# KKKSQJ/DeepLearning

Measured on NVIDIA H100. Metric: images/sec (ResNet-50 training step), higher is better.
Workload: dtype bf16

## Files before the change

### deeplearning_b200/csrc/abi_conv.cu

```cuda
#include <string.h>
#include "../../include/b200cls.h"
#include "conv_gemm.cuh"
#include "conv1x1_stream.cuh"
#include "conv_tap64.cuh"
#include "host_utils.h"
#include "wgrad_gemm.cuh"

using namespace b200;

namespace {

constexpr uint32_t kFwdDescLbo = 16, kFwdDescSbo = 1024;
constexpr uint32_t kWgDescLbo = 8192, kWgDescSbo = 1024, kWgDescKstep = 2048;

struct Box3 {
  int b1, b2, b3;
};

Box3 choose_box(long long d1, long long d2, long long d3, int P) {
  Box3 best{P, 1, 1};
  double best_cost = -1;
  for (int b1 = 1; b1 <= P; b1 <<= 1) {
    for (int b2 = 1; b1 * b2 <= P; b2 <<= 1) {
      const int b3 = P / (b1 * b2);
// ... 127 lines not shown
    }
  } else {
    *qb = Box3{bx.b1 / 4, 1, 1};
    for (int q = 0; q < 4; ++q) o1[q] = q * (bx.b1 / 4);
  }
}

int setup_output(ConvGemmParams& p, const View& dv, int N, int out_f32, const View* auxv) {
  const long long d1 = dv.dims[1], d2 = dv.dims[2], d3 = dv.dims[3];
  const Box3 bx = choose_box(d1, d2, d3, 128);
  p.box1 = bx.b1, p.box2 = bx.b2, p.box3 = bx.b3;
  p.dim1 = static_cast<int>(d1), p.dim2 = static_cast<int>(d2), p.dim3 = static_cast<int>(d3);
  p.tiles1 = static_cast<int>((d1 + bx.b1 - 1) / bx.b1);
  p.tiles2 = static_cast<int>((d2 + bx.b2 - 1) / bx.b2);
  p.tiles3 = static_cast<int>((d3 + bx.b3 - 1) / bx.b3);
  p.N = N;
  const int BN = N <= 64 ? 64 : 128;
  p.n_tiles = (N + BN - 1) / BN;
  Box3 qb;
  quarter_box(bx, &qb, p.qoff1, p.qoff2, p.qoff3);
  p.out_f32 = out_f32;
  if (dv.base != nullptr) {
    uint32_t box[4] = {out_f32 ? 32u : 64u, (uint32_t)qb.b1, (uint32_t)qb.b2, (uint32_t)qb.b3};
    int rc = out_f32 ? encode_tmap_f32(&p.d_map, dv.base, 4, dv.dims, dv.strides, box)
                     : encode_tmap_bf16(&p.d_map, dv.base, 4, dv.dims, dv.strides, box);
    if (rc) return rc;
  }
  p.has_aux_out = 0;
  if (auxv != nullptr) {
    uint32_t box[4] = {64u, (uint32_t)qb.b1, (uint32_t)qb.b2, (uint32_t)qb.b3};
    int rc = encode_tmap_bf16(&p.aux_map, auxv->base, 4, auxv->dims, auxv->strides, box);
    if (rc) return rc;
    p.has_aux_out = 1;
  }
  return OK;
}
Box3 box_of(const ConvGemmParams& p) { return Box3{p.box1, p.box2, p.box3}; }

bool bn_mask_complete(const b200_bn_mask_t* m) { return m->x_raw && m->scale && m->shift && m->stats; }
void set_bn_mask(ConvGemmParams& p, const b200_bn_mask_t* m, const View& dv) {
  p.mask_in = static_cast<const __nv_bfloat16*>(m->x_raw);
  p.ms1 = static_cast<long long>(dv.strides[1]);
  p.ms2 = static_cast<long long>(dv.strides[2]);
  p.ms3 = static_cast<long long>(dv.strides[3]);
  p.bn_scale = m->scale, p.bn_shift = m->shift, p.stats = m->stats;
}

int conv_grid(int tiles, int n_tiles, bool stats) {
  int grid = tiles < device_sm_count() ? tiles : device_sm_count();
  if (stats) grid = grid / n_tiles * n_tiles;
  return grid;
}

template <int BLOCK_N, int EPI>
int launch_conv_gemm_epi(const ConvGemmParams& q, int grid, cudaStream_t st) {
  using Cfg = ConvGemmCfg<BLOCK_N>;
  static bool configured = false;
  if (!configured) {
    B200_CHECK_CUDA(cudaFuncSetAttribute(conv_gemm_kernel<BLOCK_N, EPI>, cudaFuncAttributeMaxDynamicSharedMemorySize,
                                         Cfg::SMEM_BYTES));
    configured = true;
  }
  B200_CHECK_CUDA(launch_pdl(conv_gemm_kernel<BLOCK_N, EPI>, dim3(grid), dim3(Cfg::THREADS), Cfg::SMEM_BYTES, st, q));
  B200_LAUNCHED();
  return OK;
}

int epilogue_flags(const ConvGemmParams& p) {
  int f = 0;
  if (p.bias) f |= kEpiBias;
  if (p.colscale) f |= kEpiColscale;
  f |= (p.act & 3) << kEpiActShift;
  if (p.residual) f |= p.res_f32 ? kEpiResF32 : kEpiResBf16;
  if (p.has_aux_out) f |= kEpiAux;
  if (p.out_f32) f |= kEpiOutF32;
  if (p.out_direct) f |= kEpiDirect;
  if (p.stats) f |= kEpiStats;
  if (p.rowscale) f |= kEpiRowscale;
  if (p.affine) f = (f & ~(kEpiBias | kEpiColscale)) | kEpiAffine;
  if (p.mask_in) f |= p.bn_scale ? kEpiBnMask : kEpiMask;
  if (p.bn_scale) f &= ~kEpiStats;
  return f;
}

#define B200_EPI_LIST(X)                                                                                  \
  X(kEpiStats)                                              \
  X(0)                                                      \
  X(kEpiResBf16)                                            \
  X(kEpiBias)                                               \
  X(kEpiBias | kEpiResF32 | kEpiOutF32)                     \
  X(kEpiBias | kEpiColscale | kEpiResF32 | kEpiOutF32)      \
  X(kEpiBias | (2 << kEpiActShift) | kEpiAux)               \
  X(3 << kEpiActShift)                                      \
  X((3 << kEpiActShift) | kEpiStats)                        \
  X(kEpiOutF32)                                             \
  X(kEpiBias | kEpiOutF32)                                  \
  X(kEpiAffine | kEpiResBf16 | (1 << kEpiActShift))        \
  X(kEpiAffine | (1 << kEpiActShift))                      \
  X(kEpiAffine)                                            \
  X(kEpiMask | kEpiResBf16 | kEpiStats)                    \
  X(kEpiBnMask)                                            \
  X(kEpiBnMask | kEpiBias)

bool tap64_ok(const ConvGemmParams& p) {
  const int f = epilogue_flags(p);
  return p.N == 64 && p.n_tiles == 1 && p.k_per_tap == 64 && p.k_blocks_per_tap == 1 && !p.var_taps && !p.chan_window &&
         p.num_taps >= 2 && p.num_taps <= 9 && (f == 0 || f == kEpiStats) && p.dim1 % p.box1 == 0 && p.dim2 % p.box2 == 0 &&
         p.dim3 % p.box3 == 0;
}
template <bool kStats>
int launch_tap64(const ConvGemmParams& q, int grid, cudaStream_t st) {
  static bool configured = false;
  if (!configured) {
    B200_CHECK_CUDA(cudaFuncSetAttribute(conv_tap64_kernel<kStats>, cudaFuncAttributeMaxDynamicSharedMemorySize, kTap64SmemBytes));
    configured = true;
  }
  B200_CHECK_CUDA(launch_pdl(conv_tap64_kernel<kStats>, dim3(grid), dim3(384), kTap64SmemBytes, st, q));
  B200_LAUNCHED();
  return OK;
}

template <int BLOCK_N>
int launch_conv_gemm(const ConvGemmParams& p, cudaStream_t st) {
  const int tiles = p.tiles1 * p.tiles2 * p.tiles3 * p.n_tiles;
  const int grid = conv_grid(tiles, p.n_tiles, p.stats != nullptr);
  B200_REQUIRE(grid > 0, "conv_gemm: %d channel blocks exceed the SM count (BN statistics need grid %% n_tiles == 0)", p.n_tiles);
  ConvGemmParams q = p;
  q.desc_lbo = kFwdDescLbo;
  q.desc_sbo = kFwdDescSbo;
  if constexpr (BLOCK_N == 64) {
    if (tap64_ok(p)) return p.stats != nullptr ? launch_tap64<true>(q, grid, st) : launch_tap64<false>(q, grid, st);
  }
  switch (epilogue_flags(p)) {
#define B200_EPI_CASE(F) \
  case (F):              \
    return launch_conv_gemm_epi<BLOCK_N, (F)>(q, grid, st);
    B200_EPI_LIST(B200_EPI_CASE)
#undef B200_EPI_CASE
    default:
      return launch_conv_gemm_epi<BLOCK_N, kEpiGeneric>(q, grid, st);
  }
}


bool stream_ok(long long pixels, int K, int N) {
  return (K == 64 || K == 128 || K == 256) && N % 256 == 0 && pixels % 128 == 0 && pixels / 128 < (1LL << 30);
}
int stream_grid(long long pixels, int N) {
  const int n_tiles = N / 256;
  const long long items = pixels / 128 * n_tiles;
  int grid = items < device_sm_count() ? static_cast<int>(items) : device_sm_count();
  return grid / n_tiles * n_tiles;
}

template <int KB, int MODE>
int launch_stream(const StreamParams& q, int grid, cudaStream_t st) {
  using Cfg = StreamCfg<KB, MODE>;
  static bool configured = false;
  if (!configured) {
    B200_CHECK_CUDA(cudaFuncSetAttribute(conv1x1_stream_kernel<KB, MODE>, cudaFuncAttributeMaxDynamicSharedMemorySize,
                                         Cfg::SMEM_BYTES));
    configured = true;
  }
  B200_CHECK_CUDA(launch_pdl(conv1x1_stream_kernel<KB, MODE>, dim3(grid), dim3(Cfg::THREADS), Cfg::SMEM_BYTES, st, q));
  B200_LAUNCHED();
  return OK;
}

int run_stream(int mode, const void* a, const void* w, void* out, const void* res, const void* mask, const float* scale,
               const float* shift, float* stats, long long pixels, int K, int N, cudaStream_t st) {
  StreamParams q;
  memset(&q, 0, sizeof(q));
  int rc;
  if ((rc = encode_matrix(&q.a_map, a, K, pixels, 128))) return rc;
  if ((rc = encode_matrix(&q.b_map, w, K, N, 256))) return rc;
  if ((rc = encode_matrix(&q.out_map, out, N, pixels, 16))) return rc;
  if (res != nullptr && (rc = encode_matrix(&q.res_map, res, N, pixels, 16))) return rc;
  if (mask != nullptr && (rc = encode_matrix(&q.mask_map, mask, N, pixels, 16))) return rc;
  q.m_tiles = static_cast<int>(pixels / 128);
  q.n_tiles = N / 256;
  q.N = N;
  q.scale = scale, q.shift = shift, q.stats = stats;
  const int grid = stream_grid(pixels, N);
// ... 172 lines not shown
  const int n_tiles = (Cout + BN - 1) / BN;
  const long long tiles = m_tiles * n_tiles;
  const int grid = conv_grid(tiles > (1 << 30) ? (1 << 30) : static_cast<int>(tiles), n_tiles, true);
  return grid / n_tiles * (BN == 64 ? 8 : 4);
}

int b200_conv2d_fwd_stats_rows(int B, int H, int W, int Cout, int ksize, int stride) {
  return fwd_stats_rows(B, H, W, Cout, ksize, stride, block_n_for(Cout));
}

static int conv_fwd(const void* x, const void* w, void* y, int B, int H, int W, int Cin, int Cout, int ksize, int stride,
                    float* stats, const float* bias, int act, const void* residual, float* out_f32, long long ld_out,
                    const float* bn_scale, const float* bn_shift, int y_f32, int Cg, void* stream) {
  B200_REQUIRE(ksize == 1 || ksize == 3 || (ksize == 2 && stride == 2), "conv2d_fwd: ksize %d / stride %d unsupported", ksize, stride);
  B200_REQUIRE(stride == 1 || stride == 2, "conv2d_fwd: stride %d unsupported (1 or 2)", stride);
  B200_REQUIRE(Cin % 8 == 0 && Cout % 8 == 0, "conv2d_fwd: Cin=%d / Cout=%d must be multiples of 8", Cin, Cout);
  B200_REQUIRE(B > 0 && H > 0 && W > 0, "conv2d_fwd: empty input");
  B200_REQUIRE(stride == 1 || (H >= 2 && W >= 2), "conv2d_fwd: stride-2 needs H,W >= 2");
  B200_REQUIRE(out_f32 == nullptr || (ksize == 1 && stride == 1), "conv2d_fwd: fp32 output only for 1x1/s1");
  B200_REQUIRE((bn_scale == nullptr) == (bn_shift == nullptr), "conv2d_fwd: bn_scale and bn_shift go together");
  B200_REQUIRE(bn_scale == nullptr || (Cout % 64 == 0 && bias == nullptr && stats == nullptr && out_f32 == nullptr && act <= 1 && !y_f32),
               "conv2d_fwd + folded BN: Cout=%d must be a multiple of 64, no bias / statistics / fp32 output", Cout);
  cudaStream_t st = static_cast<cudaStream_t>(stream);
  const int Ho = out_dim(H, ksize, stride), Wo = out_dim(W, ksize, stride);
  ConvGemmParams p;
  memset(&p, 0, sizeof(p));
  int rc;
  View dv = act_view(y, B, Ho, Wo, Cout, ksize == 1 && stride == 1);
  if (out_f32 != nullptr) dv.base = nullptr;
  if ((rc = setup_output(p, dv, Cout, y_f32, nullptr))) return rc;
  const int BN = Cg ? 64 : block_n_for(Cout);
  p.n_tiles = (Cout + BN - 1) / BN;
  p.chan_window = Cg ? 1 : 0;
  p.k_per_tap = Cg ? 64 : Cin;
  p.k_blocks_per_tap = Cg ? 1 : (Cin + 63) / 64;
  p.num_taps = ksize * ksize;
  if ((rc = encode_taps(p, p.a_maps, x, B, H, W, Cin, ksize, stride, box_of(p)))) return rc;
  for (int t = 0; t < p.num_taps; ++t) p.tap_w[t] = static_cast<int8_t>(t);
  if ((rc = encode_matrix(&p.b_map, w, static_cast<long long>(p.num_taps) * p.k_per_tap, Cout, BN))) return rc;
  p.stats = stats;
  p.bias = bias;
  p.act = act;
  p.residual = residual;
  p.rs1 = static_cast<long long>(dv.strides[1]);
  p.rs2 = static_cast<long long>(dv.strides[2]);
  p.rs3 = static_cast<long long>(dv.strides[3]);
  p.out_direct = out_f32;
  p.ld_out = ld_out;
  if (bn_scale != nullptr) {
    p.affine = 1;
    p.colscale = bn_scale;
    p.bias = bn_shift;
  }
  return Cg ? launch_conv_gemm<64>(p, st) : dispatch_conv_gemm(p, Cout, st);
}

int b200_conv2d_fwd(const void* x, const void* w, void* y, int B, int H, int W, int Cin, int Cout, int ksize, int stride,
                    float* stats, const float* bias, int act, const void* residual, float* out_f32, long long ld_out,
                    const float* bn_scale, const float* bn_shift, void* stream) {
  return conv_fwd(x, w, y, B, H, W, Cin, Cout, ksize, stride, stats, bias, act, residual, out_f32, ld_out, bn_scale, bn_shift,
                  0, 0, stream);
}

int b200_conv2d_fwd_f32(const void* x, const void* w, float* y, int B, int H, int W, int Cin, int Cout, int ksize,
                        int stride, const float* bias, void* stream) {
  return conv_fwd(x, w, y, B, H, W, Cin, Cout, ksize, stride, nullptr, bias, 0, nullptr, nullptr, 0, nullptr, nullptr, 1, 0,
                  stream);
}

static int conv_dgrad(const void* dy, const void* wd, void* dx, int B, int H, int W, int Cin, int Cout, int ksize,
                      int stride, const void* residual, const b200_bn_mask_t* bn_mask, int Cg, void* stream) {
  B200_REQUIRE(ksize == 1 || ksize == 3 || (ksize == 2 && stride == 2), "conv2d_dgrad: ksize %d / stride %d unsupported", ksize, stride);
  B200_REQUIRE(stride == 1 || stride == 2, "conv2d_dgrad: stride %d unsupported", stride);
  B200_REQUIRE(Cin % 8 == 0 && Cout % 8 == 0, "conv2d_dgrad: Cin=%d / Cout=%d must be multiples of 8", Cin, Cout);
  B200_REQUIRE(bn_mask == nullptr || (stride == 1 && Cin % 64 == 0 && bn_mask_complete(bn_mask)),
               "conv2d_dgrad: the fused BatchNorm-backward reduce needs stride 1, Cin %% 64 == 0 and every bn_mask field "
               "(Cin=%d, stride=%d)", Cin, stride);
  cudaStream_t st = static_cast<cudaStream_t>(stream);
  const int Ho = out_dim(H, ksize, stride), Wo = out_dim(W, ksize, stride);
  const bool flat = (ksize == 1 && stride == 1);
  const int BN = Cg ? 64 : block_n_for(Cin);
  const int k_per_tap = Cg ? 64 : Cout;
  int rc;
  CUtensorMap b_map;
  if ((rc = encode_matrix(&b_map, wd, static_cast<long long>(ksize * ksize) * k_per_tap, Cin, BN))) return rc;
  const int nphase = (stride == 2 && ksize >= 2) ? 2 : 1;
  for (int ph = 0; ph < nphase; ++ph) {
    for (int pw = 0; pw < nphase; ++pw) {
      ConvGemmParams p;
      memset(&p, 0, sizeof(p));
      p.b_map = b_map;
      View dv = flat ? make_flat_view(dx, static_cast<long long>(B) * H * W, Cin)
                     : make_view(dx, B, H, W, Cin, stride, ph, pw);
      if ((rc = setup_output(p, dv, Cin, 0, nullptr))) return rc;
      p.n_tiles = (Cin + BN - 1) / BN;
      p.chan_window = Cg ? 1 : 0;
      p.k_per_tap = k_per_tap;
      p.k_blocks_per_tap = Cg ? 1 : (Cout + 63) / 64;
      if ((rc = encode_view(&p.a_maps[0], act_view(dy, B, Ho, Wo, Cout, flat), box_of(p)))) return rc;
      for (int i = 1; i < 4; ++i) p.a_maps[i] = p.a_maps[0];
      int nt = 0;
      if (ksize == 1) {
        p.tap_map[0] = 0, p.tap_o1[0] = 0, p.tap_o2[0] = 0, p.tap_w[0] = 0;
        nt = 1;
      } else if (stride == 1) {
        for (int kh = 0; kh < 3; ++kh)
          for (int kw = 0; kw < 3; ++kw) {
            p.tap_map[nt] = 0;
            p.tap_o1[nt] = static_cast<int8_t>(1 - kw);
            p.tap_o2[nt] = static_cast<int8_t>(1 - kh);
            p.tap_w[nt] = static_cast<int8_t>(kh * 3 + kw);
            ++nt;
          }
      } else if (ksize == 2) {
        p.tap_map[0] = 0, p.tap_o1[0] = 0, p.tap_o2[0] = 0;
        p.tap_w[0] = static_cast<int8_t>(ph * 2 + pw);
        nt = 1;
      } else {
        for (int kh = 0; kh < 3; ++kh) {
          if (((ph + 1 - kh) & 1) != 0) continue;
          for (int kw = 0; kw < 3; ++kw) {
            if (((pw + 1 - kw) & 1) != 0) continue;
            p.tap_map[nt] = 0;
            p.tap_o1[nt] = static_cast<int8_t>((pw + 1 - kw) / 2);
            p.tap_o2[nt] = static_cast<int8_t>((ph + 1 - kh) / 2);
            p.tap_w[nt] = static_cast<int8_t>(kh * 3 + kw);
            ++nt;
          }
        }
      }
      p.num_taps = nt;
      if (residual != nullptr) {
        p.residual = static_cast<const char*>(residual) + (static_cast<const char*>(dv.base) - static_cast<const char*>(dx));
        p.rs1 = static_cast<long long>(dv.strides[1]);
        p.rs2 = static_cast<long long>(dv.strides[2]);
        p.rs3 = static_cast<long long>(dv.strides[3]);
      }
      if (bn_mask != nullptr) set_bn_mask(p, bn_mask, dv);
      if ((rc = Cg ? launch_conv_gemm<64>(p, st) : dispatch_conv_gemm(p, Cin, st))) return rc;
    }
  }
  return OK;
}

int b200_conv2d_dgrad(const void* dy, const void* wd, void* dx, int B, int H, int W, int Cin, int Cout, int ksize,
                      int stride, const void* residual, const b200_bn_mask_t* bn_mask, void* stream) {
  return conv_dgrad(dy, wd, dx, B, H, W, Cin, Cout, ksize, stride, residual, bn_mask, 0, stream);
}

int b200_gemm_ex(const b200_view_t* a, const b200_view_t* out, const b200_gemm_args_t* g, void* stream) {
  B200_REQUIRE(a != nullptr && out != nullptr && g != nullptr && g->w != nullptr, "gemm_ex: null argument");
  B200_REQUIRE(g->N % 8 == 0 && g->K % 8 == 0, "gemm_ex: N=%d / K=%d must be multiples of 8", g->N, g->K);
  for (int i = 0; i < 3; ++i)
    B200_REQUIRE(a->dim[i] == out->dim[i] && a->dim[i] > 0, "gemm_ex: a/out pixel extents differ in dim %d", i);
  B200_REQUIRE(!(g->aux_out != nullptr && g->out_f32), "gemm_ex: aux_out needs a bf16 primary output");
  B200_REQUIRE(!(g->stats != nullptr && g->out_f32), "gemm_ex: stats need a bf16 output");
  auto to_view = [](const b200_view_t* v, int C) {
    View r;
    r.base = v->base;
    r.dims[0] = C;
    r.strides[0] = 1;
    for (int i = 0; i < 3; ++i) {
      r.dims[i + 1] = static_cast<uint64_t>(v->dim[i]);
      r.strides[i + 1] = static_cast<uint64_t>(v->stride[i]);
    }
    return r;
  };
  ConvGemmParams p;
  memset(&p, 0, sizeof(p));
  int rc;
  View dv = to_view(out, g->N);
  View auxv;
  if (g->aux_out) auxv = to_view(g->aux_out, g->N);
  if ((rc = setup_output(p, dv, g->N, g->out_f32, g->aux_out ? &auxv : nullptr))) return rc;
  const Box3 bx = box_of(p);
  if ((rc = encode_view(&p.a_maps[0], to_view(a, g->K), bx))) return rc;
  for (int i = 1; i < 4; ++i) p.a_maps[i] = p.a_maps[0];
  p.num_taps = 1;
  p.k_per_tap = g->K;
  p.k_blocks_per_tap = (g->K + 63) / 64;
  if ((rc = encode_matrix(&p.b_map, g->w, g->K, g->N, block_n_for(g->N)))) return rc;
  p.stats = g->stats;
  p.bias = g->bias;
  p.colscale = g->colscale;
  p.act = g->act;
  if (g->residual) {
    p.residual = g->residual->base;
    p.res_f32 = g->residual_f32;
    p.rs1 = g->residual->stride[0], p.rs2 = g->residual->stride[1], p.rs3 = g->residual->stride[2];
  }
  if (g->rowscale != nullptr) {
// ... 264 lines not shown
```

### deeplearning_b200/csrc/common.cuh

```cuda
#pragma once
#include <cuda_runtime.h>
#include <cuda_bf16.h>
#include <cuda.h>
#include <stdint.h>
#include "wgmma.cuh"

namespace b200 {

constexpr int kNumSMs = 132;

__device__ __forceinline__ void pdl_wait() { asm volatile("griddepcontrol.wait;" ::: "memory"); }

__device__ __forceinline__ uint32_t smem_u32(const void* p) {
  return static_cast<uint32_t>(__cvta_generic_to_shared(p));
}

__device__ __forceinline__ bool elect_one() {
  uint32_t pred = 0;
  asm volatile(
      "{\n\t.reg .pred P;\n\t"
      "elect.sync _|P, 0xffffffff;\n\t"
      "selp.b32 %0, 1, 0, P;\n\t}\n"
      : "=r"(pred));
  return pred != 0;
// ... 33 lines not shown
      "mbarrier.try_wait.parity.shared::cta.b64 P1, [%0], %1;\n\t"
      "@P1 bra DONE_%=;\n\t"
      "nanosleep.u32 40;\n\t"
      "bra WAIT_%=;\n\t"
      "DONE_%=:\n\t}\n" ::"r"(addr),
      "r"(parity)
      : "memory");
}

__device__ __forceinline__ void sts128(uint32_t addr, uint32_t a, uint32_t b, uint32_t c, uint32_t d) {
  asm volatile("st.shared.v4.b32 [%0], {%1, %2, %3, %4};" ::"r"(addr), "r"(a), "r"(b), "r"(c), "r"(d) : "memory");
}
__device__ __forceinline__ uint32_t lds32(uint32_t addr) {
  uint32_t v;
  asm volatile("ld.shared.b32 %0, [%1];" : "=r"(v) : "r"(addr) : "memory");
  return v;
}
__device__ __forceinline__ uint64_t f2_pack(float lo, float hi) {
  uint64_t r;
  asm("mov.b64 %0, {%1, %2};" : "=l"(r) : "f"(lo), "f"(hi));
  return r;
}
__device__ __forceinline__ void f2_unpack(uint64_t v, float& lo, float& hi) {
  asm("mov.b64 {%0, %1}, %2;" : "=f"(lo), "=f"(hi) : "l"(v));
}
__device__ __forceinline__ uint64_t f2_add(uint64_t a, uint64_t b) {
  float a0, a1, b0, b1;
  f2_unpack(a, a0, a1);
  f2_unpack(b, b0, b1);
  return f2_pack(__fadd_rn(a0, b0), __fadd_rn(a1, b1));
}
__device__ __forceinline__ uint64_t f2_mul(uint64_t a, uint64_t b) {
  float a0, a1, b0, b1;
  f2_unpack(a, a0, a1);
  f2_unpack(b, b0, b1);
  return f2_pack(__fmul_rn(a0, b0), __fmul_rn(a1, b1));
}
__device__ __forceinline__ uint64_t f2_bcast(float c) { return f2_pack(c, c); }
__device__ __forceinline__ uint64_t f2_fma(uint64_t a, uint64_t b, uint64_t c) {
  float a0, a1, b0, b1, c0, c1;
  f2_unpack(a, a0, a1);
  f2_unpack(b, b0, b1);
  f2_unpack(c, c0, c1);
  return f2_pack(__fmaf_rn(a0, b0, c0), __fmaf_rn(a1, b1, c1));
}

__device__ __forceinline__ void fence_proxy_async_smem() {
  asm volatile("fence.proxy.async.shared::cta;" ::: "memory");
}
__device__ __forceinline__ void named_bar_sync(uint32_t id, uint32_t nthreads) {
  asm volatile("bar.sync %0, %1;" ::"r"(id), "r"(nthreads) : "memory");
}

__device__ __forceinline__ void tma_prefetch_desc(const CUtensorMap* m) {
  asm volatile("prefetch.tensormap [%0];" ::"l"(reinterpret_cast<uint64_t>(m)) : "memory");
}
__device__ __forceinline__ void tma_load_2d(void* dst, const CUtensorMap* m, uint64_t* bar, int c0, int c1) {
  asm volatile(
      "cp.async.bulk.tensor.2d.shared::cluster.global.mbarrier::complete_tx::bytes [%0], [%1, {%3, %4}], [%2];" ::"r"(
          smem_u32(dst)),
      "l"(reinterpret_cast<uint64_t>(m)), "r"(smem_u32(bar)), "r"(c0), "r"(c1)
      : "memory");
}
__device__ __forceinline__ void tma_load_4d(void* dst, const CUtensorMap* m, uint64_t* bar, int c0, int c1, int c2,
                                            int c3) {
  asm volatile(
      "cp.async.bulk.tensor.4d.shared::cluster.global.mbarrier::complete_tx::bytes [%0], [%1, {%3, %4, %5, %6}], "
      "[%2];" ::"r"(smem_u32(dst)),
      "l"(reinterpret_cast<uint64_t>(m)), "r"(smem_u32(bar)), "r"(c0), "r"(c1), "r"(c2), "r"(c3)
      : "memory");
}
__device__ __forceinline__ void tma_load_3d(void* dst, const CUtensorMap* m, uint64_t* bar, int c0, int c1, int c2) {
  asm volatile(
      "cp.async.bulk.tensor.3d.shared::cluster.global.mbarrier::complete_tx::bytes [%0], [%1, {%3, %4, %5}], [%2];" ::"r"(
          smem_u32(dst)),
      "l"(reinterpret_cast<uint64_t>(m)), "r"(smem_u32(bar)), "r"(c0), "r"(c1), "r"(c2)
      : "memory");
}
__device__ __forceinline__ void tma_store_3d(const CUtensorMap* m, const void* src, int c0, int c1, int c2) {
  asm volatile("cp.async.bulk.tensor.3d.global.shared::cta.bulk_group [%0, {%2, %3, %4}], [%1];" ::"l"(
                   reinterpret_cast<uint64_t>(m)),
               "r"(smem_u32(src)), "r"(c0), "r"(c1), "r"(c2)
               : "memory");
}
__device__ __forceinline__ void tma_store_4d(const CUtensorMap* m, const void* src, int c0, int c1, int c2, int c3) {
  asm volatile("cp.async.bulk.tensor.4d.global.shared::cta.bulk_group [%0, {%2, %3, %4, %5}], [%1];" ::"l"(
                   reinterpret_cast<uint64_t>(m)),
               "r"(smem_u32(src)), "r"(c0), "r"(c1), "r"(c2), "r"(c3)
               : "memory");
}
__device__ __forceinline__ void tma_store_commit() { asm volatile("cp.async.bulk.commit_group;" ::: "memory"); }
template <int N>
__device__ __forceinline__ void tma_store_wait_read() {
  asm volatile("cp.async.bulk.wait_group.read %0;" ::"n"(N) : "memory");
}
template <int N>
__device__ __forceinline__ void tma_store_wait_all() {
  asm volatile("cp.async.bulk.wait_group %0;" ::"n"(N) : "memory");
}

__device__ __forceinline__ void wgmma_fence() { asm volatile("wgmma.fence.sync.aligned;" ::: "memory"); }
__device__ __forceinline__ void wgmma_commit() { asm volatile("wgmma.commit_group.sync.aligned;" ::: "memory"); }
template <int N>
__device__ __forceinline__ void wgmma_wait() {
  asm volatile("wgmma.wait_group.sync.aligned %0;" ::"n"(N) : "memory");
}
// ... 89 lines not shown
```

### deeplearning_b200/csrc/conv_gemm.cuh

```cuda
#pragma once
#include <cstdio>
#include "common.cuh"

namespace b200 {

constexpr int kMaxTaps = 16;

struct alignas(64) ConvGemmParams {
  CUtensorMap a_maps[4];
  CUtensorMap b_map;
  CUtensorMap d_map;
  CUtensorMap aux_map;
  int num_taps;
  int k_per_tap;
  int k_blocks_per_tap;
  int tiles1, tiles2, tiles3;
  int box1, box2, box3;
  int dim1, dim2, dim3;
  int qoff1[4], qoff2[4], qoff3[4];
  int n_tiles;
  int N;
  int8_t tap_map[kMaxTaps];
  int8_t tap_o1[kMaxTaps];
  int8_t tap_o2[kMaxTaps];
  int8_t tap_w[kMaxTaps];
  float* stats;
  const float* bias;
  const float* colscale;
  int act;
  int out_f32;
  int res_f32;
  int has_aux_out;
  const void* residual;
  long long rs1, rs2, rs3;
  const __nv_bfloat16* aux_in;
  long long as1, as2, as3;
  uint32_t desc_lbo, desc_sbo;
  float* out_direct;
  long long ld_out;
  const float* rowscale;
  int rows_per_sample;
  int var_taps;
  int kb_total;
  int16_t tap_kb[kMaxTaps];
  int32_t tap_k0[kMaxTaps];
  const __nv_bfloat16* mask_in;
  long long ms1, ms2, ms3;
  int affine;
  const float* bn_scale;
  const float* bn_shift;
  int chan_window;
};

template <int BLOCK_N>
struct ConvGemmCfg {
  static constexpr int BLOCK_M = 128;
  static constexpr int BLOCK_K = 64;
  static constexpr int A_BYTES = BLOCK_M * BLOCK_K * 2;
  static constexpr int B_BYTES = BLOCK_N * BLOCK_K * 2;
  static constexpr int STAGES = BLOCK_N == 128 ? 4 : 5;
  static constexpr int STAGE_BYTES = A_BYTES + B_BYTES;
  static constexpr int EPI_WARPS = 4;
  static constexpr int SLAB_BYTES = 32 * 128;
  static constexpr int STAGING_BYTES = EPI_WARPS * 2 * SLAB_BYTES;
  static constexpr int IMG_BYTES = BLOCK_M * BLOCK_N * 4;
  static constexpr int IMGS = BLOCK_N == 128 ? 1 : 2;
  static constexpr int BAR_BYTES = 256;
  static constexpr int SMEM_BYTES = STAGES * STAGE_BYTES + STAGING_BYTES + IMGS * IMG_BYTES + BAR_BYTES + 1024;
  static constexpr int THREADS = 512;
  static_assert(SMEM_BYTES <= 227 * 1024, "shared memory of one H100 block");
  static_assert(2 * STAGES + 2 * IMGS <= BAR_BYTES / 8, "mbarriers");
};

__device__ __forceinline__ void gelu_parts(float x, float& tail, float& e) {
  const float az = fabsf(x) * 0.70710678118654752f;
  float t;
  asm("rcp.approx.ftz.f32 %0, %1;" : "=f"(t) : "f"(fmaf(0.3275911f, az, 1.0f)));
  float poly = fmaf(1.061405429f, t, -1.453152027f);
  poly = fmaf(poly, t, 1.421413741f);
  poly = fmaf(poly, t, -0.284496736f);
  poly = fmaf(poly, t, 0.254829592f);
  asm("ex2.approx.ftz.f32 %0, %1;" : "=f"(e) : "f"(-1.4426950408889634f * az * az));
  tail = 0.5f * poly * t * e;
}
__device__ __forceinline__ float gelu_erf(float x) {
  float tail, e;
  gelu_parts(x, tail, e);
  return x * (x >= 0.f ? 1.0f - tail : tail);
}
__device__ __forceinline__ float gelu_erf_grad(float x) {
  float tail, e;
  gelu_parts(x, tail, e);
  const float cdf = x >= 0.f ? 1.0f - tail : tail;
  return fmaf(x * 0.3989422804014327f, e, cdf);
}

__device__ __forceinline__ void gelu_parts2(float x0, float x1, uint64_t& cdf, uint64_t& e) {
  const uint64_t az = f2_pack(fabsf(x0) * 0.70710678118654752f, fabsf(x1) * 0.70710678118654752f);
  float d0, d1, t0, t1, g0, g1, e0, e1, h0, h1;
  f2_unpack(f2_fma(f2_bcast(0.3275911f), az, f2_bcast(1.0f)), d0, d1);
  asm("rcp.approx.ftz.f32 %0, %1;" : "=f"(t0) : "f"(d0));
  asm("rcp.approx.ftz.f32 %0, %1;" : "=f"(t1) : "f"(d1));
  const uint64_t t = f2_pack(t0, t1);
  uint64_t poly = f2_fma(f2_bcast(1.061405429f), t, f2_bcast(-1.453152027f));
  poly = f2_fma(poly, t, f2_bcast(1.421413741f));
  poly = f2_fma(poly, t, f2_bcast(-0.284496736f));
  poly = f2_fma(poly, t, f2_bcast(0.254829592f));
  f2_unpack(f2_mul(f2_mul(az, az), f2_bcast(-1.4426950408889634f)), g0, g1);
  asm("ex2.approx.ftz.f32 %0, %1;" : "=f"(e0) : "f"(g0));
  asm("ex2.approx.ftz.f32 %0, %1;" : "=f"(e1) : "f"(g1));
  e = f2_pack(e0, e1);
  f2_unpack(f2_fma(f2_mul(f2_mul(poly, t), e), f2_bcast(-0.5f), f2_bcast(0.5f)), h0, h1);
  cdf = f2_add(f2_pack(copysignf(h0, x0), copysignf(h1, x1)), f2_bcast(0.5f));
}
__device__ __forceinline__ void gelu_erf2(float& x0, float& x1) {
  uint64_t cdf, e;
  gelu_parts2(x0, x1, cdf, e);
  f2_unpack(f2_mul(f2_pack(x0, x1), cdf), x0, x1);
}
__device__ __forceinline__ void gelu_erf_val_grad2(float& x0, float& x1, float& g0, float& g1) {
  uint64_t cdf, e;
  gelu_parts2(x0, x1, cdf, e);
  const uint64_t x = f2_pack(x0, x1);
  f2_unpack(f2_fma(f2_mul(x, f2_bcast(0.3989422804014327f)), e, cdf), g0, g1);
  f2_unpack(f2_mul(x, cdf), x0, x1);
}

#ifdef CONV_PROFILE
#define CPROF_DECL(N) long long cp_t[N] = {}; long long cp_0 = clock64(), cp_1;
#define CPROF_TICK(i) { cp_1 = clock64(); cp_t[i] += cp_1 - cp_0; cp_0 = cp_1; }
#else
#define CPROF_DECL(N)
#define CPROF_TICK(i)
#endif

template <int S>
__device__ __forceinline__ void butterfly_step(float (&px)[32], int lane) {
  const bool up = (lane & S) != 0;
#pragma unroll
  for (int i = 0; i < S; ++i) {
    const float send = up ? px[i] : px[i + S];
    const float keep = up ? px[i + S] : px[i];
    px[i] = keep + __shfl_xor_sync(0xffffffffu, send, S);
  }
}

constexpr int kEpiGeneric = -1;
constexpr int kEpiBias = 1, kEpiColscale = 2, kEpiActShift = 2 , kEpiResBf16 = 16, kEpiResF32 = 32,
              kEpiAux = 64, kEpiOutF32 = 128, kEpiDirect = 256, kEpiStats = 512,
              kEpiRowscale = 1024 ,
              kEpiAffine = 2048, kEpiMask = 4096, kEpiBnMask = 8192;

template <int BLOCK_N, int EPI = kEpiGeneric>
__global__ void __launch_bounds__(512, 1) conv_gemm_kernel(const __grid_constant__ ConvGemmParams p) {
  static_assert(BLOCK_N == 64 || BLOCK_N == 128, "64- or 128-column tiles");
  using Cfg = ConvGemmCfg<BLOCK_N>;
  constexpr int STAGES = Cfg::STAGES;
  constexpr int IMGS = Cfg::IMGS;
  extern __shared__ uint8_t smem_raw[];
  uint8_t* smem = reinterpret_cast<uint8_t*>((reinterpret_cast<uintptr_t>(smem_raw) + 1023) & ~uintptr_t(1023));
  uint8_t* stage_base = smem;
  uint8_t* staging = smem + STAGES * Cfg::STAGE_BYTES;
  uint8_t* img = staging + Cfg::STAGING_BYTES;
  uint64_t* bars = reinterpret_cast<uint64_t*>(img + IMGS * Cfg::IMG_BYTES);
  uint64_t* full_bar = bars;
  uint64_t* empty_bar = bars + STAGES;
  uint64_t* img_full = bars + 2 * STAGES;
  uint64_t* img_empty = bars + 2 * STAGES + IMGS;

  const int warp_idx = threadIdx.x >> 5;
  const int lane = threadIdx.x & 31;
  const int m_tiles = p.tiles1 * p.tiles2 * p.tiles3;
  const int num_tiles = m_tiles * p.n_tiles;
  const int num_kb = p.var_taps ? p.kb_total : p.num_taps * p.k_blocks_per_tap;

  if (warp_idx == 0 && lane == 0) {
    for (int i = 0; i < 4; ++i) tma_prefetch_desc(&p.a_maps[i]);
    tma_prefetch_desc(&p.b_map);
    tma_prefetch_desc(&p.d_map);
    for (int i = 0; i < STAGES; ++i) {
      mbar_init(&full_bar[i], 1);
      mbar_init(&empty_bar[i], 2);
    }
    for (int i = 0; i < IMGS; ++i) {
      mbar_init(&img_full[i], 8);
      mbar_init(&img_empty[i], Cfg::EPI_WARPS);
    }
    fence_mbar_init();
  }
  __syncthreads();
  pdl_wait();

  if (warp_idx < 4) {
    setmaxnreg_dec<40>();
    if (warp_idx == 0 && lane == 0) {
      int stage = 0;
      uint32_t phase = 0;
      CPROF_DECL(2)
      for (int tile = blockIdx.x; tile < num_tiles; tile += gridDim.x) {
        const int n_tile = tile % p.n_tiles;
        const int m_tile = tile / p.n_tiles;
        const int t1 = m_tile % p.tiles1;
        const int t2 = (m_tile / p.tiles1) % p.tiles2;
        const int t3 = m_tile / (p.tiles1 * p.tiles2);
        const int c1 = t1 * p.box1, c2 = t2 * p.box2, c3 = t3 * p.box3;
        int tap = 0, cb = 0;
        int kb_in_tap = p.var_taps ? p.tap_kb[0] : p.k_blocks_per_tap;
        for (int kb = 0; kb < num_kb; ++kb, ++cb) {
          if (cb == kb_in_tap) {
            cb = 0;
            ++tap;
            if (p.var_taps) kb_in_tap = p.tap_kb[tap];
          }
          const int wk = p.var_taps ? p.tap_k0[tap] + cb * 64 : p.tap_w[tap] * p.k_per_tap + cb * 64;
          CPROF_TICK(1)
          mbar_wait_backoff(&empty_bar[stage], phase ^ 1);
          CPROF_TICK(0)
          uint8_t* a_dst = stage_base + stage * Cfg::STAGE_BYTES;
          uint8_t* b_dst = a_dst + Cfg::A_BYTES;
          mbar_expect_tx(&full_bar[stage], Cfg::STAGE_BYTES);
          tma_load_4d(a_dst, &p.a_maps[p.tap_map[tap]], &full_bar[stage], p.chan_window ? n_tile * BLOCK_N : cb * 64, c1 + p.tap_o1[tap],
                      c2 + p.tap_o2[tap], c3);
          tma_load_2d(b_dst, &p.b_map, &full_bar[stage], wk, n_tile * BLOCK_N);
          if (++stage == STAGES) {
            stage = 0;
            phase ^= 1;
          }
        }
      }
#ifdef CONV_PROFILE
      if (blockIdx.x == 0) {
        const int nt = (num_tiles - 1) / gridDim.x + 1;
        printf("conv producer: wait_empty %lld issue %lld  (cycles/tile, %d tiles, %d k-blocks)\n", cp_t[0] / nt, cp_t[1] / nt, nt, num_kb);
      }
#endif
    }
  } else if (warp_idx < 12) {
    setmaxnreg_dec<112>();
    const int wg = (warp_idx - 4) >> 2;
    const uint64_t desc_a0 = make_smem_desc_sw128(smem_u32(stage_base) + wg * 8192, p.desc_lbo, p.desc_sbo);
    const uint64_t desc_b0 = make_smem_desc_sw128(smem_u32(stage_base) + Cfg::A_BYTES, p.desc_lbo, p.desc_sbo);
    int stage = 0;
    uint32_t phase = 0;
    int it = 0;
    CPROF_DECL(3)
    for (int tile = blockIdx.x; tile < num_tiles; tile += gridDim.x, ++it) {
      float acc[BLOCK_N / 2];
#pragma unroll
      for (int i = 0; i < BLOCK_N / 2; ++i) acc[i] = 0.f;
      int prev = -1;
      CPROF_TICK(2)
      for (int kb = 0; kb < num_kb; ++kb) {
        mbar_wait(&full_bar[stage], phase);
        wgmma_fence();
        const uint64_t soff = static_cast<uint64_t>(stage) * (Cfg::STAGE_BYTES >> 4);
        const uint64_t da = desc_a0 + soff, db = desc_b0 + soff;
#pragma unroll
        for (int k = 0; k < 4; ++k) Wgmma<BLOCK_N, 0, 0>::mma(acc, da + 2 * k, db + 2 * k, 1u);
        wgmma_commit();
        wgmma_wait<1>();
        if (prev >= 0 && (threadIdx.x & 127) == 0) mbar_arrive(&empty_bar[prev]);
        prev = stage;
        if (++stage == STAGES) {
          stage = 0;
          phase ^= 1;
        }
      }
      wgmma_wait<0>();
      wgmma_reg_fence(acc);
      if ((threadIdx.x & 127) == 0) mbar_arrive(&empty_bar[prev]);
      CPROF_TICK(0)
      const int b = IMGS == 1 ? 0 : it % IMGS;
      mbar_wait(&img_empty[b], ((it / IMGS) & 1) ^ 1);
      CPROF_TICK(1)
      acc_to_img<BLOCK_N>(acc, smem_u32(img + b * Cfg::IMG_BYTES), BLOCK_N, 64 * wg, 0);
      __syncwarp();
      if (lane == 0) mbar_arrive(&img_full[b]);
    }
#ifdef CONV_PROFILE
    if (blockIdx.x == 0 && lane == 0 && (warp_idx & 3) == 0) {
      const int nt = (num_tiles - 1) / gridDim.x + 1;
      printf("conv mma wg %d: main loop %lld wait img_empty %lld acc->img %lld  (cycles/tile)\n", wg, cp_t[0] / nt, cp_t[1] / nt,
             cp_t[2] / nt);
    }
#endif
  } else {
    setmaxnreg_inc<248>();
    const int q = warp_idx - 12;
    const int row = q * 32 + lane;
    const uint32_t stage_s = smem_u32(staging + q * 2 * Cfg::SLAB_BYTES);
    const uint32_t row_s = lane * 128;
    const uint32_t sw = (lane & 7) << 4;
    uint32_t stat_off[8];
#pragma unroll
    for (int m = 0; m < 8; ++m) stat_off[m] = m * 128 + ((((lane >> 2) ^ m) << 4) | ((lane & 3) << 2));
    constexpr bool G = EPI < 0;
    constexpr bool kAffine = !G && (EPI & kEpiAffine) != 0;
    constexpr bool kBnMask = !G && (EPI & kEpiBnMask) != 0;
    constexpr bool kMask = !G && (EPI & (kEpiMask | kEpiBnMask)) != 0;
    const int N = p.N;
    const float* const bias = (!kAffine && (G || (EPI & kEpiBias))) ? p.bias : nullptr;
    const float* const colscale = (!kAffine && (G || (EPI & kEpiColscale))) ? p.colscale : nullptr;
    const int act_bits = G ? p.act : ((EPI >> kEpiActShift) & 3);
    const int act = kAffine ? 0 : act_bits;
    const bool has_res = G ? (p.residual != nullptr) : ((EPI & (kEpiResBf16 | kEpiResF32)) != 0);
    const bool res_f32 = G ? (p.res_f32 != 0) : ((EPI & kEpiResF32) != 0);
    const bool has_aux = G ? (p.has_aux_out != 0) : ((EPI & kEpiAux) != 0);
    const bool out_f32 = G ? (p.out_f32 != 0) : ((EPI & kEpiOutF32) != 0);
    float* const out_direct = (G || (EPI & kEpiDirect)) ? p.out_direct : nullptr;
    float* const stats = (G || (EPI & (kEpiStats | kEpiBnMask))) ? p.stats : nullptr;
    const float* const rowscale = G ? p.rowscale : nullptr;
    const bool need_rowmap = has_res || act == 3 || kMask || out_direct != nullptr || rowscale != nullptr || p.dim1 % p.box1 != 0 ||
                             p.dim2 % p.box2 != 0 || p.dim3 % p.box3 != 0;
    const bool full_cols = (N % BLOCK_N) == 0;
    uint32_t store_counter = 0;
    const int unit_cols = out_f32 ? 32 : 64;
    const int units = BLOCK_N / unit_cols;
    const int nsub = out_f32 ? 1 : 2;
    constexpr int SLOTS = 2;
    uint64_t run_s[SLOTS], run_q[SLOTS];
    float run_x[SLOTS][2];
#pragma unroll
    for (int k = 0; k < SLOTS; ++k) run_s[k] = 0, run_q[k] = 0, run_x[k][0] = run_x[k][1] = 0.f;
    int it = 0;
    CPROF_DECL(2)
    for (int tile = blockIdx.x; tile < num_tiles; tile += gridDim.x, ++it) {
      const int b = IMGS == 1 ? 0 : it % IMGS;
      const uint32_t img_s = smem_u32(img + b * Cfg::IMG_BYTES);
      const int n_tile = tile % p.n_tiles;
      const int m_tile = tile / p.n_tiles;
      const int t1 = m_tile % p.tiles1;
      const int t2 = (m_tile / p.tiles1) % p.tiles2;
      const int t3 = m_tile / (p.tiles1 * p.tiles2);
      const int c1 = t1 * p.box1, c2 = t2 * p.box2, c3 = t3 * p.box3;
      int p1 = 0, p2 = 0, p3 = 0;
      bool row_ok = true;
      if (need_rowmap) {
        const int i1 = row % p.box1;
        const int i2 = (row / p.box1) % p.box2;
        const int i3 = row / (p.box1 * p.box2);
        p1 = c1 + i1, p2 = c2 + i2, p3 = c3 + i3;
        row_ok = (p1 < p.dim1) && (p2 < p.dim2) && (p3 < p.dim3);
      }
      const int s1 = c1 + p.qoff1[q], s2 = c2 + p.qoff2[q], s3 = c3 + p.qoff3[q];

      uint4 nx_b[4];
      float4 nx_f[8];
      uint4 nx_m[4];
      auto issue_pre = [&](int u, int h) {
        const int ncp = n_tile * BLOCK_N + u * unit_cols + h * 32;
        if (n_tile * BLOCK_N + u * unit_cols >= N || !row_ok) return;
        if (has_res) {
          const long long off = p3 * p.rs3 + p2 * p.rs2 + p1 * p.rs1 + ncp;
          if (res_f32) {
            const float4* rp = reinterpret_cast<const float4*>(static_cast<const float*>(p.residual) + off);
#pragma unroll
            for (int j = 0; j < 8; ++j)
              if (full_cols || ncp + j * 4 < N) nx_f[j] = __ldg(rp + j);
          } else {
            const uint4* rp = reinterpret_cast<const uint4*>(static_cast<const __nv_bfloat16*>(p.residual) + off);
#pragma unroll
            for (int j = 0; j < 4; ++j)
              if (full_cols || ncp + j * 8 < N) nx_b[j] = __ldg(rp + j);
          }
        }
        if (act == 3) {
          const uint4* ap = reinterpret_cast<const uint4*>(p.aux_in + p3 * p.as3 + p2 * p.as2 + p1 * p.as1 + ncp);
#pragma unroll
          for (int j = 0; j < 4; ++j)
            if (full_cols || ncp + j * 8 < N) nx_b[j] = __ldg(ap + j);
        }
        if constexpr (kMask) {
          const uint4* mp = reinterpret_cast<const uint4*>(p.mask_in + p3 * p.ms3 + p2 * p.ms2 + p1 * p.ms1 + ncp);
#pragma unroll
          for (int j = 0; j < 4; ++j)
            if (full_cols || ncp + j * 8 < N) nx_m[j] = __ldg(mp + j);
        }
      };
      if (has_res || act == 3 || kMask) issue_pre(0, 0);
      CPROF_TICK(1)
      mbar_wait(&img_full[b], (it / IMGS) & 1);
      CPROF_TICK(0)

#pragma unroll 1
      for (int u = 0; u < units; ++u) {
        const int n0 = n_tile * BLOCK_N + u * unit_cols;
        const bool chunk_live = n0 < N;
        const uint32_t buf_s = stage_s + (store_counter & 1) * Cfg::SLAB_BYTES;
        const uint32_t aux_s = stage_s + ((store_counter + 1) & 1) * Cfg::SLAB_BYTES;
        if (chunk_live && out_direct == nullptr) {
          if (lane == 0) {
            if (has_aux) tma_store_wait_read<0>(); else tma_store_wait_read<1>();
          }
          __syncwarp();
        }
#pragma unroll 1
        for (int h = 0; h < nsub; ++h) {
          uint32_t v[32];
          img_ld32(img_s, BLOCK_N, row, u * unit_cols + h * 32, v);
          if (u == units - 1 && h == nsub - 1) {
            __syncwarp();
            if (lane == 0) mbar_arrive(&img_empty[b]);
          }
          uint4 pre_b[4];
          float4 pre_f[8];
          uint4 pre_m[4];
          if (has_res || act == 3 || kMask) {
#pragma unroll
            for (int j = 0; j < 4; ++j) pre_b[j] = nx_b[j];
#pragma unroll
            for (int j = 0; j < 8; ++j) pre_f[j] = nx_f[j];
            if constexpr (kMask) {
#pragma unroll
              for (int j = 0; j < 4; ++j) pre_m[j] = nx_m[j];
            }
            if (h + 1 < nsub)
              issue_pre(u, h + 1);
            else if (u + 1 < units)
              issue_pre(u + 1, 0);
          }
          if (!chunk_live) continue;
          const int nc = n0 + h * 32;
          float f[32];
#pragma unroll
          for (int j = 0; j < 32; ++j) f[j] = __uint_as_float(v[j]);
          if constexpr (kAffine) {
#pragma unroll
            for (int j = 0; j < 8; ++j) {
              const float4 s4 = __ldg(reinterpret_cast<const float4*>(p.colscale + nc) + j);
              const float4 b4 = __ldg(reinterpret_cast<const float4*>(p.bias + nc) + j);
              f2_unpack(f2_fma(f2_pack(f[j * 4 + 0], f[j * 4 + 1]), f2_pack(s4.x, s4.y), f2_pack(b4.x, b4.y)), f[j * 4 + 0], f[j * 4 + 1]);
              f2_unpack(f2_fma(f2_pack(f[j * 4 + 2], f[j * 4 + 3]), f2_pack(s4.z, s4.w), f2_pack(b4.z, b4.w)), f[j * 4 + 2], f[j * 4 + 3]);
            }
          }
          if (bias != nullptr) {
            if (full_cols) {
#pragma unroll
              for (int j = 0; j < 8; ++j) {
                const float4 b4 = __ldg(reinterpret_cast<const float4*>(bias + nc) + j);
                f2_unpack(f2_add(f2_pack(f[j * 4 + 0], f[j * 4 + 1]), f2_pack(b4.x, b4.y)), f[j * 4 + 0], f[j * 4 + 1]);
                f2_unpack(f2_add(f2_pack(f[j * 4 + 2], f[j * 4 + 3]), f2_pack(b4.z, b4.w)), f[j * 4 + 2], f[j * 4 + 3]);
              }
            } else {
#pragma unroll
              for (int j = 0; j < 32; ++j) f[j] += (nc + j < N) ? __ldg(bias + nc + j) : 0.0f;
// ... 237 lines not shown
```

Measured before the change: 8791.

## Add halo-box mode for 3x3 stride-1 convs with resident weights

Adds a HALO variant of the conv GEMM kernel for 64-channel 3x3 stride-1 convolutions. Each tile loads three 8x10x2 halo boxes, one per horizontal offset, and reuses each box across the three vertical taps by offsetting the smem descriptor. All nine weight taps are loaded into shared memory once per block instead of being re-streamed per k-block. This cuts TMA traffic and shared-memory fill per tile, and the mask input is L2-prefetched. In exchange the epilogue staging drops to one slab and one accumulator image, which reduces overlap between epilogue stores and MMA.

```diff
diff --git a/deeplearning_b200/csrc/abi_conv.cu b/deeplearning_b200/csrc/abi_conv.cu
--- a/deeplearning_b200/csrc/abi_conv.cu
+++ b/deeplearning_b200/csrc/abi_conv.cu
@@ -203,16 +203,16 @@
   return grid;
 }
 
-template <int BLOCK_N, int EPI>
+template <int BLOCK_N, int EPI, bool HALO = false>
 int launch_conv_gemm_epi(const ConvGemmParams& q, int grid, cudaStream_t st) {
-  using Cfg = ConvGemmCfg<BLOCK_N>;
+  using Cfg = ConvGemmCfg<BLOCK_N, HALO>;
   static bool configured = false;
   if (!configured) {
-    B200_CHECK_CUDA(cudaFuncSetAttribute(conv_gemm_kernel<BLOCK_N, EPI>, cudaFuncAttributeMaxDynamicSharedMemorySize,
+    B200_CHECK_CUDA(cudaFuncSetAttribute(conv_gemm_kernel<BLOCK_N, EPI, HALO>, cudaFuncAttributeMaxDynamicSharedMemorySize,
                                          Cfg::SMEM_BYTES));
     configured = true;
   }
-  B200_CHECK_CUDA(launch_pdl(conv_gemm_kernel<BLOCK_N, EPI>, dim3(grid), dim3(Cfg::THREADS), Cfg::SMEM_BYTES, st, q));
+  B200_CHECK_CUDA(launch_pdl(conv_gemm_kernel<BLOCK_N, EPI, HALO>, dim3(grid), dim3(Cfg::THREADS), Cfg::SMEM_BYTES, st, q));
   B200_LAUNCHED();
   return OK;
 }
@@ -271,6 +271,27 @@
   return OK;
 }
 
+bool halo_ok(const ConvGemmParams& p) {
+  const int f = epilogue_flags(p);
+  if (!(p.N == 64 && p.n_tiles == 1 && p.k_per_tap == 64 && p.k_blocks_per_tap == 1 && !p.var_taps && !p.chan_window &&
+        p.num_taps == 9 && (f == kEpiStats || f == kEpiBnMask)))
+    return false;
+  if (p.box1 != 8 || p.box2 != 8 || p.box3 != 2 || p.dim1 % 8 != 0 || p.dim2 % 8 != 0 || p.dim3 % 2 != 0) return false;
+  for (int t = 0; t < 9; ++t) {
+    if (p.tap_map[t] != 0 || p.tap_o1[t] != p.tap_o1[t % 3] || p.tap_o2[t] != p.tap_o2[t - t % 3] || p.tap_o2[t] < -1 ||
+        p.tap_o2[t] > 1)
+      return false;
+  }
+  return true;
+}
+int set_halo(ConvGemmParams& p, const View& v) {
+  if (!halo_ok(p)) return OK;
+  const uint32_t box[4] = {64, 8, 10, 2};
+  const int rc = encode_tmap_bf16(&p.a_maps[1], v.base, 4, v.dims, v.strides, box);
+  p.halo = rc == OK;
+  return rc;
+}
+
 template <int BLOCK_N>
 int launch_conv_gemm(const ConvGemmParams& p, cudaStream_t st) {
   const int tiles = p.tiles1 * p.tiles2 * p.tiles3 * p.n_tiles;
@@ -280,6 +301,10 @@
   q.desc_lbo = kFwdDescLbo;
   q.desc_sbo = kFwdDescSbo;
   if constexpr (BLOCK_N == 64) {
+    if (p.halo) {
+      return epilogue_flags(p) == kEpiStats ? launch_conv_gemm_epi<64, kEpiStats, true>(q, grid, st)
+                                            : launch_conv_gemm_epi<64, kEpiBnMask, true>(q, grid, st);
+    }
     if (tap64_ok(p)) return p.stats != nullptr ? launch_tap64<true>(q, grid, st) : launch_tap64<false>(q, grid, st);
   }
   switch (epilogue_flags(p)) {
@@ -558,6 +583,7 @@
     p.colscale = bn_scale;
     p.bias = bn_shift;
   }
+  if (!Cg && ksize == 3 && stride == 1 && (rc = set_halo(p, make_view(x, B, H, W, Cin, 1, 0, 0)))) return rc;
   return Cg ? launch_conv_gemm<64>(p, st) : dispatch_conv_gemm(p, Cout, st);
 }
 
@@ -643,6 +669,7 @@
         p.rs3 = static_cast<long long>(dv.strides[3]);
       }
       if (bn_mask != nullptr) set_bn_mask(p, bn_mask, dv);
+      if (!Cg && ksize == 3 && stride == 1 && (rc = set_halo(p, act_view(dy, B, Ho, Wo, Cout, false)))) return rc;
       if ((rc = Cg ? launch_conv_gemm<64>(p, st) : dispatch_conv_gemm(p, Cin, st))) return rc;
     }
   }
diff --git a/deeplearning_b200/csrc/common.cuh b/deeplearning_b200/csrc/common.cuh
--- a/deeplearning_b200/csrc/common.cuh
+++ b/deeplearning_b200/csrc/common.cuh
@@ -109,6 +109,9 @@
   asm volatile("bar.sync %0, %1;" ::"r"(id), "r"(nthreads) : "memory");
 }
 
+__device__ __forceinline__ void l2_prefetch_bulk(const void* src, uint32_t bytes) {
+  asm volatile("cp.async.bulk.prefetch.L2.global [%0], %1;" ::"l"(reinterpret_cast<uint64_t>(src)), "r"(bytes) : "memory");
+}
 __device__ __forceinline__ void tma_prefetch_desc(const CUtensorMap* m) {
   asm volatile("prefetch.tensormap [%0];" ::"l"(reinterpret_cast<uint64_t>(m)) : "memory");
 }
diff --git a/deeplearning_b200/csrc/conv_gemm.cuh b/deeplearning_b200/csrc/conv_gemm.cuh
--- a/deeplearning_b200/csrc/conv_gemm.cuh
+++ b/deeplearning_b200/csrc/conv_gemm.cuh
@@ -47,29 +47,36 @@
   const __nv_bfloat16* mask_in;
   long long ms1, ms2, ms3;
   int affine;
+  int halo;
   const float* bn_scale;
   const float* bn_shift;
   int chan_window;
 };
 
-template <int BLOCK_N>
+template <int BLOCK_N, bool HALO = false>
 struct ConvGemmCfg {
+  static_assert(!HALO || BLOCK_N == 64, "the halo mode runs 64-column tiles");
   static constexpr int BLOCK_M = 128;
   static constexpr int BLOCK_K = 64;
   static constexpr int A_BYTES = BLOCK_M * BLOCK_K * 2;
   static constexpr int B_BYTES = BLOCK_N * BLOCK_K * 2;
-  static constexpr int STAGES = BLOCK_N == 128 ? 4 : 5;
-  static constexpr int STAGE_BYTES = A_BYTES + B_BYTES;
+  static constexpr int HALO_TAPS = 9;
+  static constexpr int HALO_BOX_BYTES = 2 * 10 * 8 * 128;
+  static constexpr int W_BYTES = HALO ? HALO_TAPS * B_BYTES : 0;
+  static constexpr int STAGES = HALO ? 5 : (BLOCK_N == 128 ? 4 : 5);
+  static constexpr int STAGE_BYTES = HALO ? HALO_BOX_BYTES : A_BYTES + B_BYTES;
   static constexpr int EPI_WARPS = 4;
   static constexpr int SLAB_BYTES = 32 * 128;
-  static constexpr int STAGING_BYTES = EPI_WARPS * 2 * SLAB_BYTES;
+  static constexpr int SLABS = HALO ? 1 : 2;
+  static constexpr int STAGING_BYTES = EPI_WARPS * SLABS * SLAB_BYTES;
   static constexpr int IMG_BYTES = BLOCK_M * BLOCK_N * 4;
-  static constexpr int IMGS = BLOCK_N == 128 ? 1 : 2;
+  static constexpr int IMGS = (BLOCK_N == 128 || HALO) ? 1 : 2;
   static constexpr int BAR_BYTES = 256;
-  static constexpr int SMEM_BYTES = STAGES * STAGE_BYTES + STAGING_BYTES + IMGS * IMG_BYTES + BAR_BYTES + 1024;
+  static constexpr int SMEM_BYTES = W_BYTES + STAGES * STAGE_BYTES + STAGING_BYTES + IMGS * IMG_BYTES + BAR_BYTES + 1024;
   static constexpr int THREADS = 512;
   static_assert(SMEM_BYTES <= 227 * 1024, "shared memory of one H100 block");
-  static_assert(2 * STAGES + 2 * IMGS <= BAR_BYTES / 8, "mbarriers");
+  static_assert(2 * STAGES + 2 * IMGS + 1 <= BAR_BYTES / 8, "mbarriers");
+  static_assert(!HALO || STAGES >= 4, "the halo ring must hold more than one tile's boxes");
 };
 
 __device__ __forceinline__ void gelu_parts(float x, float& tail, float& e) {
@@ -151,22 +158,25 @@
               kEpiRowscale = 1024 ,
               kEpiAffine = 2048, kEpiMask = 4096, kEpiBnMask = 8192;
 
-template <int BLOCK_N, int EPI = kEpiGeneric>
+template <int BLOCK_N, int EPI = kEpiGeneric, bool HALO = false>
 __global__ void __launch_bounds__(512, 1) conv_gemm_kernel(const __grid_constant__ ConvGemmParams p) {
   static_assert(BLOCK_N == 64 || BLOCK_N == 128, "64- or 128-column tiles");
-  using Cfg = ConvGemmCfg<BLOCK_N>;
+  static_assert(!HALO || (EPI >= 0 && (EPI & kEpiAux) == 0), "the halo mode's single staging slab has no room for a second output");
+  using Cfg = ConvGemmCfg<BLOCK_N, HALO>;
   constexpr int STAGES = Cfg::STAGES;
   constexpr int IMGS = Cfg::IMGS;
   extern __shared__ uint8_t smem_raw[];
   uint8_t* smem = reinterpret_cast<uint8_t*>((reinterpret_cast<uintptr_t>(smem_raw) + 1023) & ~uintptr_t(1023));
-  uint8_t* stage_base = smem;
-  uint8_t* staging = smem + STAGES * Cfg::STAGE_BYTES;
+  uint8_t* w_res = smem;
+  uint8_t* stage_base = smem + Cfg::W_BYTES;
+  uint8_t* staging = stage_base + STAGES * Cfg::STAGE_BYTES;
   uint8_t* img = staging + Cfg::STAGING_BYTES;
   uint64_t* bars = reinterpret_cast<uint64_t*>(img + IMGS * Cfg::IMG_BYTES);
   uint64_t* full_bar = bars;
   uint64_t* empty_bar = bars + STAGES;
   uint64_t* img_full = bars + 2 * STAGES;
   uint64_t* img_empty = bars + 2 * STAGES + IMGS;
+  uint64_t* w_full = bars + 2 * STAGES + 2 * IMGS;
 
   const int warp_idx = threadIdx.x >> 5;
   const int lane = threadIdx.x & 31;
@@ -175,7 +185,11 @@
   const int num_kb = p.var_taps ? p.kb_total : p.num_taps * p.k_blocks_per_tap;
 
   if (warp_idx == 0 && lane == 0) {
-    for (int i = 0; i < 4; ++i) tma_prefetch_desc(&p.a_maps[i]);
+    if constexpr (HALO) {
+      tma_prefetch_desc(&p.a_maps[1]);
+    } else {
+      for (int i = 0; i < 4; ++i) tma_prefetch_desc(&p.a_maps[i]);
+    }
     tma_prefetch_desc(&p.b_map);
     tma_prefetch_desc(&p.d_map);
     for (int i = 0; i < STAGES; ++i) {
@@ -186,6 +200,7 @@
       mbar_init(&img_full[i], 8);
       mbar_init(&img_empty[i], Cfg::EPI_WARPS);
     }
+    if constexpr (HALO) mbar_init(w_full, 1);
     fence_mbar_init();
   }
   __syncthreads();
@@ -193,7 +208,32 @@
 
   if (warp_idx < 4) {
     setmaxnreg_dec<40>();
-    if (warp_idx == 0 && lane == 0) {
+    if (HALO && warp_idx == 0 && lane == 0) {
+      mbar_expect_tx(w_full, Cfg::HALO_TAPS * Cfg::B_BYTES);
+      for (int t = 0; t < Cfg::HALO_TAPS; ++t) tma_load_2d(w_res + t * Cfg::B_BYTES, &p.b_map, w_full, p.tap_w[t] * p.k_per_tap, 0);
+      int stage = 0;
+      uint32_t phase = 0;
+      for (int tile = blockIdx.x; tile < num_tiles; tile += gridDim.x) {
+        const int t1 = tile % p.tiles1;
+        const int t2 = (tile / p.tiles1) % p.tiles2;
+        const int t3 = tile / (p.tiles1 * p.tiles2);
+        for (int j = 0; j < 3; ++j) {
+          mbar_wait_backoff(&empty_bar[stage], phase ^ 1);
+          mbar_expect_tx(&full_bar[stage], Cfg::STAGE_BYTES);
+          tma_load_4d(stage_base + stage * Cfg::STAGE_BYTES, &p.a_maps[1], &full_bar[stage], 0, t1 * p.box1 + p.tap_o1[j],
+                      t2 * p.box2 - 1, t3 * p.box3);
+          if (++stage == STAGES) {
+            stage = 0;
+            phase ^= 1;
+          }
+        }
+        if constexpr ((EPI & (kEpiMask | kEpiBnMask)) != 0) {
+          const __nv_bfloat16* m = p.mask_in + t3 * 2 * p.ms3 + t2 * 8 * p.ms2 + t1 * 8 * p.ms1;
+#pragma unroll 1
+          for (int r = 0; r < 16; ++r) l2_prefetch_bulk(m + (r >> 3) * p.ms3 + (r & 7) * p.ms2, static_cast<uint32_t>(7 * p.ms1 + 64) * 2u);
+        }
+      }
+    } else if (warp_idx == 0 && lane == 0) {
       int stage = 0;
       uint32_t phase = 0;
       CPROF_DECL(2)
@@ -240,6 +280,9 @@
     const int wg = (warp_idx - 4) >> 2;
     const uint64_t desc_a0 = make_smem_desc_sw128(smem_u32(stage_base) + wg * 8192, p.desc_lbo, p.desc_sbo);
     const uint64_t desc_b0 = make_smem_desc_sw128(smem_u32(stage_base) + Cfg::A_BYTES, p.desc_lbo, p.desc_sbo);
+    const uint64_t desc_h0 = make_smem_desc_sw128(smem_u32(stage_base) + wg * (Cfg::HALO_BOX_BYTES / 2), p.desc_lbo, p.desc_sbo);
+    const uint64_t desc_w0 = make_smem_desc_sw128(smem_u32(w_res), p.desc_lbo, p.desc_sbo);
+    if constexpr (HALO) mbar_wait(w_full, 0);
     int stage = 0;
     uint32_t phase = 0;
     int it = 0;
@@ -250,20 +293,47 @@
       for (int i = 0; i < BLOCK_N / 2; ++i) acc[i] = 0.f;
       int prev = -1;
       CPROF_TICK(2)
-      for (int kb = 0; kb < num_kb; ++kb) {
-        mbar_wait(&full_bar[stage], phase);
-        wgmma_fence();
-        const uint64_t soff = static_cast<uint64_t>(stage) * (Cfg::STAGE_BYTES >> 4);
-        const uint64_t da = desc_a0 + soff, db = desc_b0 + soff;
-#pragma unroll
-        for (int k = 0; k < 4; ++k) Wgmma<BLOCK_N, 0, 0>::mma(acc, da + 2 * k, db + 2 * k, 1u);
-        wgmma_commit();
-        wgmma_wait<1>();
-        if (prev >= 0 && (threadIdx.x & 127) == 0) mbar_arrive(&empty_bar[prev]);
-        prev = stage;
-        if (++stage == STAGES) {
-          stage = 0;
-          phase ^= 1;
+      if constexpr (HALO) {
+        int slot[3];
+        uint32_t par[3];
+#pragma unroll
+        for (int j = 0; j < 3; ++j) {
+          slot[j] = stage, par[j] = phase;
+          if (++stage == STAGES) {
+            stage = 0;
+            phase ^= 1;
+          }
+        }
+#pragma unroll
+        for (int t = 0; t < Cfg::HALO_TAPS; ++t) {
+          const int j = t % 3;
+          if (t < 3) mbar_wait(&full_bar[slot[j]], par[j]);
+          wgmma_fence();
+          const uint64_t da = desc_h0 + static_cast<uint64_t>((slot[j] * Cfg::STAGE_BYTES + (p.tap_o2[t] + 1) * 1024) >> 4);
+          const uint64_t db = desc_w0 + static_cast<uint64_t>(t * (Cfg::B_BYTES >> 4));
+#pragma unroll
+          for (int k = 0; k < 4; ++k) Wgmma<BLOCK_N, 0, 0>::mma(acc, da + 2 * k, db + 2 * k, 1u);
+          wgmma_commit();
+          wgmma_wait<1>();
+          if (t >= 7 && (threadIdx.x & 127) == 0) mbar_arrive(&empty_bar[slot[t - 7]]);
+        }
+        prev = slot[2];
+      } else {
+        for (int kb = 0; kb < num_kb; ++kb) {
+          mbar_wait(&full_bar[stage], phase);
+          wgmma_fence();
+          const uint64_t soff = static_cast<uint64_t>(stage) * (Cfg::STAGE_BYTES >> 4);
+          const uint64_t da = desc_a0 + soff, db = desc_b0 + soff;
+#pragma unroll
+          for (int k = 0; k < 4; ++k) Wgmma<BLOCK_N, 0, 0>::mma(acc, da + 2 * k, db + 2 * k, 1u);
+          wgmma_commit();
+          wgmma_wait<1>();
+          if (prev >= 0 && (threadIdx.x & 127) == 0) mbar_arrive(&empty_bar[prev]);
+          prev = stage;
+          if (++stage == STAGES) {
+            stage = 0;
+            phase ^= 1;
+          }
         }
       }
       wgmma_wait<0>();
@@ -288,7 +358,7 @@
     setmaxnreg_inc<248>();
     const int q = warp_idx - 12;
     const int row = q * 32 + lane;
-    const uint32_t stage_s = smem_u32(staging + q * 2 * Cfg::SLAB_BYTES);
+    const uint32_t stage_s = smem_u32(staging + q * Cfg::SLABS * Cfg::SLAB_BYTES);
     const uint32_t row_s = lane * 128;
     const uint32_t sw = (lane & 7) << 4;
     uint32_t stat_off[8];
@@ -386,11 +456,11 @@
       for (int u = 0; u < units; ++u) {
         const int n0 = n_tile * BLOCK_N + u * unit_cols;
         const bool chunk_live = n0 < N;
-        const uint32_t buf_s = stage_s + (store_counter & 1) * Cfg::SLAB_BYTES;
-        const uint32_t aux_s = stage_s + ((store_counter + 1) & 1) * Cfg::SLAB_BYTES;
+        const uint32_t buf_s = stage_s + (store_counter % Cfg::SLABS) * Cfg::SLAB_BYTES;
+        const uint32_t aux_s = stage_s + ((store_counter + 1) % Cfg::SLABS) * Cfg::SLAB_BYTES;
         if (chunk_live && out_direct == nullptr) {
           if (lane == 0) {
-            if (has_aux) tma_store_wait_read<0>(); else tma_store_wait_read<1>();
+            if (has_aux) tma_store_wait_read<0>(); else tma_store_wait_read<Cfg::SLABS - 1>();
           }
           __syncwarp();
         }
```

Result: no change. 8870 (median of 6 runs) (+0.9%).
